# pcubillos/pyratbay

Measured on AMD Instinct MI355X. Metric: spectra/sec (1e5 wavenumbers x 80 layers), higher is better.
Workload: dtype f64; 1 GPU; 1e5 wavenumbers x 80 layers, 1e5 synthetic lines, transit; nwave=100001, nlayers=80, nlines=100000, wnosamp=180, voigt_grid=nlor=100 ndop=50 extent=300 cutoff=25, voigt_table_bytes=1448022784, parallelism=single GPU, 2 independent spectra in flight on 2 HIP streams, ranks=1, priming_spectra_in_init=32

## Files before the change

### include/pbhip.h

```cpp
#ifndef PBHIP_H
#define PBHIP_H

#include <stdint.h>

#ifdef __cplusplus
extern "C" {
#endif

#define PB_OK 0
#define PB_ERR_ARG (-1)
#define PB_ERR_HIP (-2)
#define PB_ERR_UNSUPPORTED (-3)
#define PB_ERR_NOMEM (-4)

const char *pb_last_error(void);
int pb_version(void);
int pb_device_count(int *count);
int pb_set_device(int device);

typedef struct pb_timer pb_timer;

int pb_timer_create(pb_timer **out, int max_stages);
int pb_timer_start(pb_timer *t, const char *first_stage, void *stream);
int pb_timer_mark(pb_timer *t, const char *name, const char *next_stage, void *stream);
// ... 42 lines not shown
int pb_lbl_set_isoiext(pb_lbl *p, const int32_t *isoiext_h);
int pb_lbl_set_ethresh(pb_lbl *p, double ethresh);
int pb_lbl_set_gather_mode(pb_lbl *p, int mode);
int pb_lbl_last_gather_mode(const pb_lbl *p, int *mode);
int pb_lbl_set_concurrency(pb_lbl *p, int n);
int pb_lbl_set_record_budget(pb_lbl *p, int64_t bytes);
int pb_lbl_last_chunks(const pb_lbl *p, int *chunks);
int pb_lbl_extinction(pb_lbl *p, double *ext_d, int64_t wbegin, int64_t wcount,
                      const double *temp_d, const double *dens_d, const double *isoz_d,
                      int64_t z_iso_stride, int64_t z_layer_stride, int nlayers, int add,
                      void *stream);
int pb_lbl_last_state(pb_lbl *p, int32_t *ofactor_h, double *kmax_h, int nlayers,
                      int nrows, void *stream);
int pb_lbl_last_layer_kinds(pb_lbl *p, int32_t *resident_h, int32_t *block_h, int nlayers,
                            void *stream);
int pb_lbl_extinction_begin(pb_lbl *p, double *ext_d, int64_t wbegin, int64_t wcount,
                            const double *temp_d, const double *dens_d, const double *isoz_d,
                            int64_t z_iso_stride, int64_t z_layer_stride, int nlayers, int add,
                            void *stream);
int pb_lbl_kmax_buffer(pb_lbl *p, void **kmax_d, int64_t *count);
int pb_lbl_extinction_end(pb_lbl *p, void *stream);
int pb_lbl_last_work(pb_lbl *p, int64_t work[3], void *stream);
int pb_lbl_last_table_samples(pb_lbl *p, int64_t *samples, void *stream);
int pb_lbl_timing_begin(pb_lbl *p, int max_launches);
int pb_lbl_timing_end(pb_lbl *p, double *total_ms, int *launches);
void pb_lbl_destroy(pb_lbl *p);

int pb_interp_ec(double *extinction_d, const double *etable_d, const double *ttable_d,
                 const double *temperatures_d, const double *density_d, int nmol,
                 int ntemp, int nlayers, int nwave, int lay1, int lay2, int per_mol,
// ... 550 lines not shown
```

### pyratbay_amd/_capi.py

```python
import ctypes as C
import os

import numpy as np

_HERE = os.path.dirname(os.path.abspath(__file__))
LIBPATH = os.environ.get('PB_LIBPBHIP') or os.path.join(_HERE, 'libpbhip.so')

PB_OK = 0


class PbError(RuntimeError):
    pass


_lib = None

vp = C.c_void_p
i32, i64, u64, f64 = C.c_int, C.c_int64, C.c_uint64, C.c_double

_PROTOS = {
    'pb_version': [],
    'pb_device_count': [C.POINTER(C.c_int)],
    'pb_set_device': [i32],
    'pb_timer_create': [C.POINTER(vp), i32],
# ... 19 lines not shown
    'pb_lbl_create': [C.POINTER(vp), vp, vp, vp, i32, vp, i32, vp, vp, i32, vp, vp, vp, vp,
                      i32, f64, f64, i32, i32],
    'pb_lbl_set_isoiext': [vp, vp],
    'pb_lbl_set_ethresh': [vp, f64],
    'pb_lbl_set_gather_mode': [vp, i32],
    'pb_lbl_set_concurrency': [vp, i32],
    'pb_lbl_set_record_budget': [vp, i64],
    'pb_lbl_last_chunks': [vp, C.POINTER(i32)],
    'pb_lbl_last_gather_mode': [vp, C.POINTER(i32)],
    'pb_lbl_extinction': [vp, vp, i64, i64, vp, vp, vp, i64, i64, i32, i32, vp],
    'pb_lbl_extinction_begin': [vp, vp, i64, i64, vp, vp, vp, i64, i64, i32, i32, vp],
    'pb_lbl_kmax_buffer': [vp, C.POINTER(vp), C.POINTER(i64)],
    'pb_lbl_extinction_end': [vp, vp],
    'pb_lbl_last_state': [vp, vp, vp, i32, i32, vp],
    'pb_lbl_last_layer_kinds': [vp, vp, vp, i32, vp],
    'pb_lbl_last_work': [vp, C.POINTER(i64 * 3), vp],
    'pb_lbl_last_table_samples': [vp, C.POINTER(i64), vp],
    'pb_lbl_timing_begin': [vp, i32],
    'pb_lbl_timing_end': [vp, C.POINTER(f64), C.POINTER(i32)],
    'pb_lbl_destroy': [vp],
    'pb_interp_ec': [vp, vp, vp, vp, vp, i32, i32, i32, i32, i32, i32, i32, vp],
    'pb_interp_ec_set': [vp, vp, vp, vp, vp, i32, i32, i32, i32, i32, i32, i32, vp],
    'pb_transit_path': [vp, vp, i32, i32, i32, vp],
    'pb_iso_partition': [vp, i64, i64, vp, i64, vp, i32, vp, i32, vp, vp],
    'pb_resample_cross_section': [vp, vp, vp, vp, vp, vp, vp, i32, i32, i32, i32, i32, i32, i32,
                                  i32, vp],
    'pb_interp_ec_batch_work_doubles': [i32, i32],
    'pb_interp_ec_batch_plan': [vp, i32, i32, i32, i32, i32, i32, i32],
    'pb_interp_ec_batch': [vp, vp, vp, vp, vp, vp, i32, i32, i32, i32, i32, vp],
    'pb_transit_work_doubles': [i32, i32, i32, i32, i32],
# ... 107 lines not shown
    'pb_lbl_set_dyn_predict': [vp, i32],
    'pb_table_transit_supported': [i32, i32, i32, i32, i32, i32],
    'pb_table_transit_work_doubles': [i32, i32, i32, i32, i32],
    'pb_table_transit_batch': [vp, vp, vp, vp, vp, vp, vp, f64, i32, i32, f64, i32, i32, i32, i32,
                               i32, vp, vp],
}
_RESTYPES = {'pb_transit_work_doubles': C.c_int64, 'pb_two_stream_batch_work_doubles': C.c_int64,
             'pb_two_stream_net_work_doubles': C.c_int64, 'pb_two_stream_net_parts': C.c_int,
             'pb_weighted_quantiles_work_doubles': C.c_int64,
             'pb_lm_work_doubles': C.c_int64,
             'pb_weighted_quantiles_resident_rows': C.c_int,
             'pb_band_contribution_work_doubles': C.c_int64,
             'pb_interp_ec_batch_work_doubles': C.c_int64,
             'pb_interp_ec_batch_cont_work_doubles': C.c_int64, 'pb_table_transit_work_doubles': C.c_int64,
             'pb_table_transit_supported': C.c_int, 'pb_voigt_destroy': None, 'pb_lines_destroy': None, 'pb_lbl_destroy': None,
             'pb_voigt_device_bytes': i64, 'pb_timer_destroy': None}
_NO_CHECK = set(_RESTYPES) | {'pb_version', 'pb_roctx_available'}


def exported_names():
    return sorted(list(_PROTOS) + ['pb_last_error'])


def experiments():
    return hasattr(lib(), 'pb_table_transit_batch')


def _preload_torch_hip_runtime():
    import torch
    cand = os.path.join(os.path.dirname(torch.__file__), 'lib', 'libamdhip64.so')
    if os.path.exists(cand):
# ... 62 lines not shown
```

### pyratbay_amd/csrc/pb_ext_args.h

```cpp
#pragma once

#include <cstdint>

#include "pb_common.h"
#include "pb_internal.h"

namespace pbx {

#ifdef PB_EXPERIMENTS
constexpr bool kExp = true;
#else
constexpr bool kExp = false;
#endif

constexpr int kBlock = 256;
constexpr int kChunks = 2;
constexpr int kLaneSamples = 2;
constexpr int kChunk = 64 * kLaneSamples;
constexpr int kWaveSpan = kChunks * kChunk;
constexpr int kTile = 4 * kWaveSpan;
constexpr int kRecs = 4;
static_assert(kTile <= kPmPad, "table padding must cover one tile");
static_assert(kTile < 65536, "window coordinates are packed in 16 bits");

constexpr int kLongLenBits = 14;
constexpr int kChunkRow = 1024;
constexpr int kRecLayers = 4;

constexpr int kBinSamples = 256;
constexpr int kStagePad = 256;
constexpr int kStageSpan = 256;
constexpr int kStageRowMax = 1024;

constexpr int kStagedWaves = 8;
constexpr int kStagedThreads = kStagedWaves * 64;
constexpr int64_t kStagedSub = kStagedWaves * kStageSpan;

constexpr int kResWaves = 8;
constexpr int kResThreads = kResWaves * 64;
constexpr int kResStrips = 2;
constexpr int kResTile = kResThreads * kResStrips;
constexpr int kResCapDefault = 8192;
static_assert(kResTile < 65536, "window coordinates are packed in 16 bits");

constexpr int kWvTile = 2048;
constexpr int kWvRowMax = 384;

// ... 22 lines not shown
    const int32_t *psize;
    const int32_t *pindex;
    const double *doppler;
    const double *lorentz;
    int ndop, nlor, osamp;
    const double *lwn, *elow, *gf;
    const int32_t *lid;
    const int32_t *gfirst, *gcount, *giown;
    const int64_t *iso_gstart;
    const int32_t *ph_first, *ph_count, *ph_iown;
    const int64_t *ph_start;
    const int32_t *ph_bin;
    int ph_nbins;
    int rowcap;
    int rowlds;
    const int32_t *ph_iso;
    const int32_t *giso;
    const int32_t *rk_first, *rk_count, *rk_iown, *rk_iso;
    const double *rk_lwn, *rk_elow, *rk_gf;
    const double *g_lead;
    int use_records;
    int64_t ngroups;
    int64_t rec_flo, rec_fhi;
    int kmax_local;
    const int32_t *wm_lo[2];
    const int32_t *wm_off[2];
    int wm_n[2];
    int wm_lds;
    int64_t wm_total[2];
    int32_t *ls_resident;
// ... 211 lines not shown
```

### pyratbay_amd/csrc/pb_ext_gather.hip

```cpp
#include <algorithm>
#include <climits>
#include <cmath>
#include <vector>

#include "pb_ext_plan.h"

using namespace pbx;

namespace {

template <int RS, int NW>
__global__ __launch_bounds__(NW * 64) void k_ext_resample(LblArgs a)
{
    constexpr int NT = NW * 64;
    constexpr int kTileRS = (NW / RS) * kWaveSpan;
    static_assert(NW % RS == 0, "wavefronts must divide evenly into record shares");
    __shared__ double s_k[NT];
    __shared__ unsigned s_off[NT];
    __shared__ unsigned s_win[NT];

    int tile, layer;
    decode_block(a, tile, layer);
    if (layer < 0 || (a.res_cap > 0 && a.ls_resident[layer]))
        return;
// ... 164 lines not shown
            }
        }
    }
    double *dst = a.ext + ((int64_t)layer * a.nrows + row) * a.wcount + (t0 - a.wbegin);
#pragma unroll
    for (int s = 0; s < kChunks; s++) {
        const int j = rlo + s * kChunk + 2 * lane;
        if (j < rhi)
            dst[j] = acc[s][0];
        if (j + 1 < rhi)
            dst[j + 1] = acc[s][1];
    }
}


template <int NW, int S, bool kDma, int kProbe = 0, int kIssue = 0>
__global__ __launch_bounds__(NW * 64, 8) void k_ext_staged(LblArgs a)
{
    constexpr int kThreads = NW * 64;
    constexpr int kSub = NW * kStageSpan;
    constexpr int kT = S * kSub;
    constexpr int kRowRegs = (kStageRowMax + kThreads - 1) / kThreads;
    static_assert(kT < 65536, "window coordinates are packed in 16 bits");
    extern __shared__ __align__(16) unsigned char smem[];
    const int osamp = a.osamp;
    double *s_row = reinterpret_cast<double *>(smem);
    struct __align__(16) Rec {
        double k;
        int qoff;
        unsigned win;
    };
// ... 27 lines not shown
            zsplit = e & 0xff;
        } else {
            layer = a.nlayers - 1 - unit / a.nsplit;
            zsplit = unit % a.nsplit;
        }
    }
    if (layer < 0 || (a.res_cap > 0 && a.ls_resident[layer]) || (a.wave_cap > 0 && a.ls_wave[layer]))
        return;
    const int nsp = a.tsplit ? a.tsplit[tile] : a.lsplit ? a.lsplit[layer] : a.nsplit;
    if (zsplit >= nsp)
        return;
    const int row = blockIdx.y;
    const int tid = threadIdx.x;
    const int lane = tid & 63;
    const int wave = __builtin_amdgcn_readfirstlane(tid >> 6);
    unsigned long long pc[21] = {0, 0, 0, 0, 0, 0, 0, 0, 0, 0, 0, 0, 0, 0, 0, 0, 0, 0, 0, 0, 0};
    auto tick = [&]() -> unsigned long long {
        if constexpr (kProbe == 4)
            return (unsigned long long)__builtin_amdgcn_s_memtime();
        return 0ull;
    };
    unsigned long long real_birth = 0;
    if constexpr (kProbe == 4) {
        real_birth = (unsigned long long)__builtin_amdgcn_s_memrealtime();
        const unsigned long long c0 = tick();
        const unsigned long long c1 = tick();
        const unsigned long long c2 = tick();
        pc[16] = (c2 - c0) + 0 * c1;
        pc[17] = 1;
    }
    const unsigned long long t_birth = tick();
// ... 19 lines not shown
    if (a.accumulate) {
#pragma unroll
        for (int u = 0; u < S; u++)
#pragma unroll
            for (int c = 0; c < 4; c++) {
                const int j = rlo + u * kSub + c * 64 + lane;
                if (j < tlen)
                    acc[u][c] = dst[j];
            }
    }
    for (int i = tid; i < kNB * rowspan + kStagePad; i += kThreads)
        s_row[i] = 0.0;

    double ring[kDma ? 1 : 2 * kRowRegs];
    int rowlim = a.rowlds;
    const unsigned row_lds0 = (unsigned)(size_t)(__attribute__((address_space(3))) char *)(
        reinterpret_cast<char *>(s_row + kStagePad));
    auto dma_desc = [&](unsigned long long d, int buf, int c_lo, int c_hi,
                        unsigned long long tref = 0) {
        const unsigned dlo = (unsigned)__builtin_amdgcn_readfirstlane((int)d);
        const unsigned dhi = (unsigned)__builtin_amdgcn_readfirstlane((int)(d >> 32));
        const long long first = ((long long)(dhi & 0xffu) << 32) | dlo;
        const int len = (int)((dhi >> 8) & 0xfffu), mlo = (int)(dhi >> 20);
        const unsigned long long base = (unsigned long long)(a.pm + first);
        typedef int v4i __attribute__((ext_vector_type(4)));
        v4i rsrc;
        rsrc.x = __builtin_amdgcn_readfirstlane((int)base);
        rsrc.y = __builtin_amdgcn_readfirstlane((int)((base >> 32) & 0xffffu));
        rsrc.z = __builtin_amdgcn_readfirstlane(len * 8);
        rsrc.w = 0x00020000;
        int voff = (2 * lane - (mlo & ~1)) * 8;
        unsigned dst = (unsigned)__builtin_amdgcn_readfirstlane((int)(row_lds0 + buf * rowspan * 8));
        if constexpr (kProbe == 4) {
            if (tref)
                pc[20] += tick() - tref;
        }
        voff += 1024 * c_lo;
        dst += 1024 * (unsigned)c_lo;
        for (int c = c_lo; c < c_hi && c * 128 < rowlim; c++) {
            unsigned keep;
            asm volatile("s_nop 4\n\t"
                         "s_mov_b32 %0, m0\n\t"
                         "s_mov_b32 m0, %1\n\t"
                         "s_nop 0\n\t"
                         "buffer_load_dwordx4 %2, %3, 0 offen lds\n\t"
                         "s_mov_b32 m0, %0"
                         : "=&s"(keep)
// ... 56 lines not shown
        const int64_t flo = t0 * osamp - reach, fhi = (tend - 1) * osamp + reach;

        __syncthreads();
        const int cell0 = a.li_ilor[li] * a.ndop;
        for (int d = tid; d < a.ndop; d += kThreads) {
            s_cbase[d] = a.pm_base[cell0 + d];
            s_csize[d] = a.psize[cell0 + d];
            s_cstride[d] = a.pm_stride[cell0 + d];
        }
        {
            const int lim = min(a.rowlds, a.li_rowmax[li]);
            if (lim != rowlim) {
                for (int i = tid; i < kNB * rowspan + kStagePad; i += kThreads)
                    s_row[i] = 0.0;
                rowlim = lim;
            }
        }
        const int nch = a.nch_max > 1
                            ? (min(a.rowcap, a.li_rowmax[li]) + kChunkRow - 1) / kChunkRow
                            : 1;
        const int nvirt = osamp * nch;
        const int per = (nvirt + kThreads - 1) / kThreads;
        int mine = 0;
        for (int r = 0; r < per; r++) {
            const int pv = tid * per + r;
            const int p = pv / nch, c = pv - p * nch;
            if (pv < nvirt && ((nsp > 1 && p * nsp / osamp != zsplit) ||
                               iso * osamp + p < a.key_lo || iso * osamp + p >= a.key_hi)) {
                s_phs[pv] = 0;
                s_cum[pv] = 0;
// ... 199 lines not shown
                            hi = mid;
                        else
                            lo = mid + 1;
                    }
                    hits[u] = slo < tlen ? (unsigned)first | ((unsigned)(lo - first) << 16) : 0u;
                }
            };
            auto walk = [&](int sg, int buf) {
                if ((sg & 63) == 0) {
                    const unsigned long long tf = tick();
                    find_hits(sg);
                    pc[3] += tick() - tf;
                }
                bool any = false;
                const char *rowp = reinterpret_cast<const char *>(
                    s_row + kStagePad + buf * rowspan + rlo + lane);
#pragma unroll
                for (int u = 0; u < S; u++) {
                    const unsigned h = (unsigned)__builtin_amdgcn_readlane((int)hits[u], sg & 63);
                    if (h < 0x10000u)
                        continue;
                    if constexpr (kProbe == 4) {
                        pc[12] += h >> 16;
                        any = true;
                    }
                    const int first = (int)(h & 0xffff);
                    const int last = first + (int)(h >> 16);
                    const char *rs = rowp + (size_t)u * kSub * 8;
                    const double2 *recs = reinterpret_cast<const double2 *>(s_rec);
                    auto visit = [&](const double2 raw) {
                        const double k = raw.x;
// ... 92 lines not shown
                    unsigned long long dn = s_desc[min(nseg - 1, 1)];
                    dma_desc(s_desc[0], 0, wave * kPer, wave * kPer + kPer);
                    __builtin_amdgcn_s_waitcnt(0x0f70);
                    __syncthreads();
                    for (int sg = 0; sg < nseg; sg++) {
                        const unsigned long long dcur = dn;
                        dn = s_desc[min(nseg - 1, sg + 2)];
                        if (sg + 1 < nseg)
                            dma_desc(dcur, (sg + 1) & 1, wave * kPer, wave * kPer + kPer);
                        walk(sg, sg & 1);
                        __builtin_amdgcn_s_waitcnt(0x0f70);
                        __syncthreads();
                    }
                    continue;
                }
                unsigned long long ta = tick();
                if (wave == 0)
                    dma_row(0, 0);
                __builtin_amdgcn_s_waitcnt(0x0f70);
                __syncthreads();
                if constexpr (kProbe == 4) {
                    const unsigned long long tb = tick();
                    pc[8] += tb - ta;
                    ta = tb;
                }
                for (int sg = 0; sg < nseg; sg++) {
                    if (sg + 1 < nseg && wave == ((sg + 1) & (NW - 1)))
                        dma_row(sg + 1, (sg + 1) & 1, ta);
                    if constexpr (kProbe == 4) {
                        const unsigned long long tb = tick();
                        if (sg + 1 < nseg && wave == ((sg + 1) & (NW - 1))) {
                            pc[4] += tb - ta;
                            pc[19] += 1;
                        } else {
                            pc[18] += tb - ta;
                        }
                        ta = tb;
                        const unsigned long long f0 = pc[3];
                        walk(sg, sg & 1);
                        const unsigned long long tc = tick();
                        pc[5] += (tc - ta) - (pc[3] - f0);
                        __builtin_amdgcn_s_waitcnt(0x0f70);
                        const unsigned long long td = tick();
                        pc[6] += td - tc;
                        __syncthreads();
                        ta = tick();
                        pc[7] += ta - td;
                        pc[10] += 1;
                        continue;
                    }
                    walk(sg, sg & 1);
                    __builtin_amdgcn_s_waitcnt(0x0f70);
                    __syncthreads();
                }
            } else if (nseg > 0) {
                run(std::integral_constant<int, 2>(), std::integral_constant<int, kRowRegs>());
            }
        }
    }

    const unsigned long long t_out = tick();
#pragma unroll
    for (int u = 0; u < S; u++) {
#pragma unroll
        for (int c = 0; c < 4; c++) {
            const int j = rlo + u * kSub + c * 64 + lane;
            if (j < tlen)
                dst[j] = acc[u][c];
        }
    }
    if constexpr (kProbe == 4) {
        const unsigned long long t_end = tick();
        pc[14] += t_end - t_out;
        pc[9] = t_end - t_birth;
        pc[15] = (unsigned long long)__builtin_amdgcn_s_memrealtime() - real_birth;
        if (lane == 0 && a.probe)
            for (int i = 0; i < 21; i++)
                atomicAdd(&a.probe[(int64_t)layer * 24 + i], pc[i]);
    }
}

__global__ __launch_bounds__(kResThreads) void k_ext_resident(LblArgs a)
{
    extern __shared__ __align__(16) unsigned char smem[];
    struct __align__(16) Rec {
        double k;
        int off;
        unsigned win;
    };
    double *s_prof = reinterpret_cast<double *>(smem);
    const int zslot = a.res_cap;
    Rec *s_rec = reinterpret_cast<Rec *>(s_prof + a.res_cap + 2);
// ... 326 lines not shown
        return;
    const int64_t j = (int64_t)blockIdx.x * kBlock + threadIdx.x;
    if (j >= per_layer)
        return;
    const int64_t i = (int64_t)layer * per_layer + j;
    double v = ext[i];
    for (int p = 0; p < nparts; p++)
        v += part[(int64_t)p * n + i];
    ext[i] = v;
}

}

namespace pbx {

GatherKernel staged_kernel(int S, bool dma)
{
    return dma ? (S == 4   ? k_ext_staged<kStagedWaves, 4, true>
                  : S == 2 ? k_ext_staged<kStagedWaves, 2, true>
                           : k_ext_staged<kStagedWaves, 1, true>)
               : (S == 4   ? k_ext_staged<kStagedWaves, 4, false>
                  : S == 2 ? k_ext_staged<kStagedWaves, 2, false>
                           : k_ext_staged<kStagedWaves, 1, false>);
}

int allow_lds(const void *kern, size_t lds)
{
    if (lds > 64 * 1024)
        PB_HIP(hipFuncSetAttribute(kern, hipFuncAttributeMaxDynamicSharedMemorySize, (int)lds));
    return PB_OK;
}

// ... 97 lines not shown

static int exp_stage_probe_begin(LblArgs &a, const GatherPlan &g, const Tuning &tn,
                                 GatherKernel *kern, hipStream_t s)
{
    const int e = tn.stage_probe;
    if (g.S != 2 || !g.dma)
        return PB_OK;
    if (e >= 1 && e <= 3)
        *kern = e == 1   ? k_ext_staged<kStagedWaves, 2, true, 1>
                : e == 2 ? k_ext_staged<kStagedWaves, 2, true, 2>
                         : k_ext_staged<kStagedWaves, 2, true, 3>;
    if (e >= 11 && e <= 12)
        *kern = e == 11 ? k_ext_staged<kStagedWaves, 2, true, 0, 1>
                        : k_ext_staged<kStagedWaves, 2, true, 0, 2>;
    if (e == 4) {
        *kern = k_ext_staged<kStagedWaves, 2, true, 4>;
        PB_HIP(hipMalloc(&a.probe, (size_t)a.nlayers * 24 * 8));
        PB_HIP(hipMemsetAsync(a.probe, 0, (size_t)a.nlayers * 24 * 8, s));
    }
    return PB_OK;
}

static int exp_stage_probe_end(LblArgs &a, hipStream_t s)
{
    if (!a.probe)
        return PB_OK;
    std::vector<unsigned long long> h((size_t)a.nlayers * 24);
    PB_HIP(hipMemcpyAsync(h.data(), a.probe, h.size() * 8, hipMemcpyDeviceToHost, s));
    std::vector<int32_t> rowmax((size_t)a.nlayers * a.niso);
    PB_HIP(hipMemcpyAsync(rowmax.data(), a.li_rowmax, rowmax.size() * 4,
                          hipMemcpyDeviceToHost, s));
    PB_HIP(hipStreamSynchronize(s));
    (void)hipFree(a.probe);
    a.probe = nullptr;
    for (int layer = 0; layer < a.nlayers; layer++) {
        fprintf(stderr, "STAGE_PROBE layer %d rowmax %d :", layer,
                rowmax[(size_t)layer * a.niso]);
        for (int i = 0; i < 21; i++)
            fprintf(stderr, " %llu", h[(size_t)layer * 24 + i]);
        fprintf(stderr, "\n");
    }
    return PB_OK;
}
#else
static inline int exp_stage_probe_begin(LblArgs &, const GatherPlan &, const Tuning &,
                                        GatherKernel *, hipStream_t) { return PB_OK; }
static inline int exp_stage_probe_end(LblArgs &, hipStream_t) { return PB_OK; }
#endif

static int tile_split_table(pb_lbl *p, const LblArgs &a, const GatherPlan &g, const Tuning &tn,
                            int nsplit, hipStream_t s)
{
    const pb_voigt *v = p->voigt;
// ... 108 lines not shown
    }
    if (deep > 0) {
        if (int rc = layer_split_table(p, nlayers, nsplit, deep, deep_split, s))
            return rc;
        a.unit_tab = p->d_unit_tab;
        a.lsplit = p->d_lsplit;
        a.nunits = p->ut_units;
    }
    const int nunits = deep > 0 ? p->ut_units : nlayers * nsplit;
    a.nsplit = nsplit;
    if (int rc = ensure_part(p, a, deep > 0 ? deep_split : nsplit, s))
        return rc;
    a.ntiles = pb::div_up(wcount, g.S * kStagedSub);
    const int unit_groups = (nunits + 7) / 8;
    dim3 grid((unsigned)(8 * a.ntiles * unit_groups), a.nrows);
    GatherKernel kern = staged_kernel(g.S, g.dma);
    if (int rc = exp_stage_probe_begin(a, g, tn, &kern, s))
        return rc;
    if (int rc = allow_lds(reinterpret_cast<const void *>(kern), g.lds))
        return rc;
    if (int rc = exp_launch_wave(a, nunits, s))
        return rc;
    kern<<<grid, kStagedThreads, g.lds, s>>>(a);
    if (int rc = exp_stage_probe_end(a, s))
        return rc;
    const int32_t *resident = a.res_cap > 0 ? a.ls_resident : nullptr;
    const int64_t per_layer = (int64_t)a.nrows * wcount, n = nlayers * per_layer;
    if (deep > 0) {
        PB_LAUNCH_CHECK();
        dim3 cgrid((unsigned)pb::div_up(per_layer, kBlock), nlayers);
        k_combine_layer_parts<<<cgrid, kBlock, 0, s>>>(a.ext, p->part, p->d_lsplit, per_layer, n,
// ... 55 lines not shown
```

### pyratbay_amd/csrc/pb_ext_plan.h

```cpp
#pragma once

#include <vector>

#include "pb_ext_args.h"

struct pb_lbl {
    pb_voigt *voigt = nullptr;
    pb_lines *lines = nullptr;
    int nwave = 0, nmol = 0, niso = 0, ndivs = 0, max_layers = 0, resolution = 0;
    int nrows_sep = 1;
    double cutoff = 0, ethresh = 0, wnstep = 0, wn0 = 0;
    std::vector<int32_t> isoiext;
    double *d_wn = nullptr, *d_molrad = nullptr, *d_molmass = nullptr, *d_isomass = nullptr,
           *d_isoratio = nullptr;
    int32_t *d_divisors = nullptr, *d_isoimol = nullptr, *d_isoiext = nullptr;
    int32_t *ls_ofactor = nullptr, *ls_scale = nullptr, *li_ilor = nullptr, *li_hmax = nullptr;
    int32_t *li_rowmax = nullptr, *li_hlo = nullptr, *li_hhi = nullptr;
    int64_t *ls_dnwn = nullptr;
    double *ls_dwnstep = nullptr, *li_alphad = nullptr, *li_dens = nullptr, *li_z = nullptr;
    double *ls_quot = nullptr;
    double *li_invz = nullptr;
    unsigned long long *kmax_bits = nullptr;
    int kmax_rows = 0;
    int32_t *ph_first = nullptr, *ph_count = nullptr, *ph_iown = nullptr;
// ... 31 lines not shown
    bool res_look_pending = false;
    size_t record_budget = (size_t)96 << 30;
    int last_chunks = 0;
    int32_t *d_unit_tab = nullptr, *d_lsplit = nullptr;
    size_t ut_bytes = 0, ls_bytes = 0;
    int32_t *d_tsplit = nullptr;
    int32_t *pos2ph = nullptr;
    bool ts_sparse = false;
    int64_t ts_key[4] = {-1, -1, -1, -1};
    int ts_max = 0;
    size_t ts_bytes = 0;
    int ut_key[4] = {-1, -1, -1, -1};
    int ut_units = 0;
    int concurrency = 1;
    int gather_mode = 0;
    int last_gather = 0;
    double stage_threshold = 8.0;
    std::vector<hipEvent_t> ev;
    int ev_used = 0;
    int64_t *unit_cap = nullptr;
    size_t unit_cap_bytes = 0;
    int64_t cap_key[5] = {-1, -1, -1, -1, -1};
    pbx::VRec *vrec = nullptr;
    pbx::VSeg *vseg = nullptr;
    int32_t *vrnd = nullptr;
    size_t vrec_alloc = 0;
    pbx::UnitHdr *uhdr = nullptr;
    size_t uhdr_bytes = 0;
    struct Pending {
        double *ext;
// ... 33 lines not shown
    std::vector<int32_t> h_ofactor, h_ilor, h_divisors, h_isoimol, h_isoiext0;
    std::vector<double> h_wn, h_molrad, h_molmass, h_isomass, h_isoratio;
};

namespace pbx {

using Call = pb_lbl::Pending;
using GatherKernel = void (*)(LblArgs);

struct Tuning {
    int experiment = 0;
    bool dma = true;
    bool no_long_rows = false;
    int stage_s = 0;
    int stage_split = 0;
    bool poison = false;
    bool budget_set = false;
    size_t budget = 0;
    bool rec_soa = false;
    int wave = -1;
    bool res_dyn_off = false;
    bool rec_layers_1 = false;
    bool no_window_map = false;
    size_t wm_lds_cap = 48 * 1024;
    int scatter_t = 512;
    int rounds_geom = 2;
    bool deep_set = false;
    double deep_frac = 0.0;
    int deep_factor = 2;
    bool tile_split_off = false;
// ... 28 lines not shown
    int fmt = 0;
};

int64_t group_reach(const pb_voigt *v, double cutoff, double ownstep);
int64_t groups_in_reach(const pb_lines *l, int niso, int64_t flo, int64_t fhi);
int ensure_bytes(void **ptr, size_t *have, size_t need, hipStream_t s, bool sync_first,
                 const char *what);
int64_t plane_bytes(const LblArgs &a);
int cap_split_to_planes(int n, int64_t plane, int least = 1);
int ensure_part(pb_lbl *p, LblArgs &a, int nplanes, hipStream_t s);
int lbl_extinction(pb_lbl *p, const Call &c, void *stream, int phase);
int launch_layer_state(const LblArgs &a, hipStream_t s);
int launch_kmax(const LblArgs &a, hipStream_t s);
size_t records_lds(const LblArgs &a, int per);
int launch_records(const LblArgs &a, int fmt, int per, dim3 grid, size_t lds, hipStream_t s);
GatherKernel staged_kernel(int S, bool dma);
int allow_lds(const void *kern, size_t lds);
int launch_staged(pb_lbl *p, LblArgs &a, const GatherPlan &g, const Tuning &tn, hipStream_t s);
int launch_global(LblArgs &a, const Tuning &tn, hipStream_t s);
int launch_resident(LblArgs &a, hipStream_t s);
int launch_linterp(LblArgs &a, hipStream_t s);
int lbl_resolution_dyn(pb_lbl *p, LblArgs &a, const Call &c, const Tuning &tn, hipStream_t s);

#ifdef PB_EXPERIMENTS
int exp_launch_scatter(LblArgs &a, const Tuning &tn, hipStream_t s);
int exp_launch_rounds(pb_lbl *p, LblArgs &a, const GatherPlan &g, const Tuning &tn, hipStream_t s);
int exp_launch_wave(const LblArgs &a, int nunits, hipStream_t s);
#else
static inline int exp_launch_scatter(LblArgs &, const Tuning &, hipStream_t) { return PB_OK; }
static inline int exp_launch_rounds(pb_lbl *, LblArgs &, const GatherPlan &, const Tuning &,
                                    hipStream_t) { return PB_OK; }
// ... 5 lines not shown
```

### pyratbay_amd/csrc/pb_ext_resolution.hip

```cpp
#include <algorithm>
#include <vector>

#include "pb_ext_plan.h"

using namespace pbx;

namespace {

__global__ __launch_bounds__(kBlock) void k_ext_linterp(LblArgs a)
{
    struct __align__(16) RecA {
        double k;
        int64_t start;
    };
    struct __align__(16) RecB {
        int inoff, half2, mn, mx;
    };
    __shared__ RecA s_ra[kBlock + 4];
    __shared__ RecB s_rb[kBlock + 4];

    int tile, layer;
    decode_block(a, tile, layer);
    if (layer < 0)
        return;
// ... 181 lines not shown
    for (int32_t x : p->h_divisors)
        if (x <= f && f % x == 0)
            divs.push_back(x);
    const int64_t dn = 1 + (l->onwn - 1) / f;
    std::vector<double> wn((size_t)dn);
    for (int64_t i = 0; i < dn; i++)
        wn[(size_t)i] = l->own0 + (double)(i * f) * l->ownstep;
    rc = pb_lbl_create(&d.plan, d.voigt, p->lines, wn.data(), (int)dn, divs.data(),
                       (int)divs.size(), p->h_molrad.data(), p->h_molmass.data(), p->nmol,
                       p->h_isoimol.data(), p->h_isomass.data(), p->h_isoratio.data(),
                       p->h_isoiext0.data(), p->niso, p->cutoff, p->ethresh, 0, p->max_layers);
    if (rc)
        return rc;
    if (!getenv("PB_GATHER"))
        d.plan->gather_mode = 2;
    p->dyn.push_back(d);
    *out = &p->dyn.back();
    return PB_OK;
}

int lbl_resolution_dyn(pb_lbl *p, LblArgs &a, const Call &c, const Tuning &tn, hipStream_t s)
{
    const pb_lines *l = p->lines;
    const int nlayers = c.nlayers;
    const int64_t wbegin = c.wbegin, wcount = c.wcount;
    PB_REQUIRE(l->onwn < (1LL << 30), "pb_lbl_extinction: fine grid of %lld samples exceeds 2^30",
               (long long)l->onwn);
    if (int rc = launch_layer_state(a, s))
        return rc;
    const size_t nstate = (size_t)nlayers * (1 + p->niso);
// ... 290 lines not shown
```

### pyratbay_amd/csrc/pb_extinction.hip

```cpp
#include <algorithm>
#include <climits>
#include <cmath>
#include <cstdlib>
#include <new>
#include <vector>

#include "pb_ext_plan.h"

using namespace pbx;

namespace {

__global__ __launch_bounds__(kBlock) void k_poison_records(Rec16 *rec16, int64_t n16, Rec32 *rec32,
                                                          int64_t n32, double *rec_k,
                                                          int32_t *rec_i32, int64_t nsoa)
{
    const int64_t stride = (int64_t)gridDim.x * kBlock;
    for (int64_t i = (int64_t)blockIdx.x * kBlock + threadIdx.x; i < n16; i += stride) {
        Rec16 r;
        r.k = 1e300;
        r.ulo = 0;
        r.lc = 0xfffu;
        rec16[i] = r;
    }
// ... 382 lines not shown
static Tuning read_tuning()
{
    Tuning t;
    auto is_zero = [](const char *name) {
        const char *e = getenv(name);
        return e && atoi(e) == 0;
    };
    if (const char *e = getenv("PB_EXPERIMENT"))
        t.experiment = atoi(e);
    t.dma = !is_zero("PB_STAGE_DMA");
    t.no_long_rows = getenv("PB_NO_LONG_ROWS") != nullptr;
    if (const char *e = getenv("PB_STAGE_S"))
        t.stage_s = atoi(e) >= 4 ? 4 : atoi(e) >= 2 ? 2 : 1;
    if (const char *e = getenv("PB_STAGE_SPLIT"))
        t.stage_split = std::max(1, std::min(8, atoi(e)));
    if (const char *e = getenv("PB_POISON_RECORDS"))
        t.poison = atoi(e) != 0;
    if (const char *e = getenv("PB_RECORD_BUDGET")) {
        t.budget_set = true;
        t.budget = (size_t)atoll(e);
    }
    t.rec_soa = getenv("PB_REC_SOA") != nullptr;
    t.res_dyn_off = is_zero("PB_RES_DYN");
    if (const char *e = getenv("PB_REC_LAYERS"))
        t.rec_layers_1 = atoi(e) == 1;
    t.no_window_map = getenv("PB_NO_WINDOW_MAP") != nullptr;
    if (const char *e = getenv("PB_WM_LDS_CAP"))
        t.wm_lds_cap = (size_t)atol(e);
    if (const char *e = getenv("PB_STAGE_DEEP")) {
        t.deep_set = true;
// ... 418 lines not shown

static int run_chunked(pb_lbl *p, LblArgs &a, const GatherPlan &g, hipStream_t s)
{
    const int nlayers = a.nlayers;
    if (int rc = launch_kmax(a, s))
        return rc;
    const bool timed = p->ev_used + 2 <= (int)p->ev.size();
    if (timed)
        PB_HIP(hipEventRecord(p->ev[p->ev_used], s));
    const int per = kRecLayers;
    const size_t rlds = records_lds(a, per) + 8;
    PB_REQUIRE(rlds <= 64 * 1024, "pb_lbl_extinction: %zu B of LDS for the record kernel", rlds);
    a.ntiles = pb::div_up(a.wcount, g.S * kStagedSub);
    const int unit_groups = (nlayers + 7) / 8;
    dim3 ggrid((unsigned)(8 * a.ntiles * unit_groups), a.nrows);
    GatherKernel kern = staged_kernel(g.S, g.dma);
    if (int rc = allow_lds(reinterpret_cast<const void *>(kern), g.lds))
        return rc;
    for (size_t c = 0; c < g.chunks.size(); c++) {
        a.grp_lo = g.chunks[c].g_lo;
        a.grp_hi = g.chunks[c].g_hi;
        a.rec_pitch = std::max<int64_t>(1, a.grp_hi - a.grp_lo);
        a.key_lo = g.chunks[c].key_lo;
        a.key_hi = g.chunks[c].key_hi;
        a.accumulate = c > 0 ? 1 : 0;
        if (a.grp_hi > a.grp_lo) {
            dim3 rgrid(pb::div_up(a.grp_hi - a.grp_lo, kBlock), pb::div_up(nlayers, per));
            if (int rc = launch_records(a, g.fmt, per, rgrid, rlds, s))
                return rc;
        }
        kern<<<ggrid, kStagedThreads, g.lds, s>>>(a);
// ... 121 lines not shown
        if (int rc = pb_voigt_ensure_flat(p->voigt, s))
            return rc;
    const Tuning tn = read_tuning();
    LblArgs a = fill_args(p, c);
    a.kmax_local = phase != 0 ? 1 : 0;
    a.experiment = tn.experiment;

    GatherPlan g = plan_gather(p, a, tn, phase);
    resident_probe(p, g, s, phase);
    if (g.rc)
        return g.rc;
    const bool chunked = !g.chunks.empty();
    p->last_chunks = (int)g.chunks.size();
    a.nch_max = g.nch_max;
    a.rowlds = g.rowlds;
    a.res_cap = g.resident && !chunked ? p->res_cap : 0;
    if (int rc = bind_records(p, a, g, tn, s))
        return rc;

    bool dyn_fall = false;
    if (p->resolution && p->gather_mode == 6 && phase == 0 && l->ngroups > 0 &&
        l->onwn > 2 * (int64_t)p->voigt->osamp && !tn.res_dyn_off) {
        const int rc = lbl_resolution_dyn(p, a, c, tn, s);
        if (!(rc == PB_ERR_UNSUPPORTED && p->dyn_runs == 0)) {
            if (rc != PB_OK || !p->dyn_fallback)
                return rc;
            dyn_fall = true;
            a.lskip = p->d_ok;
        }
    }
// ... 118 lines not shown
        PB_HIP(hipMemcpy(kmax_h, p->kmax_bits, (size_t)nlayers * nrows * 8,
                         hipMemcpyDeviceToHost));
    return PB_OK;
}

int pb_lbl_last_layer_kinds(pb_lbl *p, int32_t *resident_h, int32_t *block_h, int nlayers,
                            void *stream)
{
    PB_REQUIRE(p, "pb_lbl_last_layer_kinds: null handle");
    PB_REQUIRE(nlayers >= 1 && nlayers <= p->max_layers, "pb_lbl_last_layer_kinds: bad sizes");
    PB_HIP(hipStreamSynchronize(pb::as_stream(stream)));
    if (resident_h)
        PB_HIP(hipMemcpy(resident_h, p->ls_resident, (size_t)nlayers * 4, hipMemcpyDeviceToHost));
    if (block_h)
        PB_HIP(hipMemcpy(block_h, p->ls_block, (size_t)nlayers * 4, hipMemcpyDeviceToHost));
    return PB_OK;
}

#ifdef PB_EXPERIMENTS
int pb_lbl_last_wave_layers(pb_lbl *p, int32_t *wave_h, int nlayers, void *stream)
{
    PB_REQUIRE(p && wave_h, "pb_lbl_last_wave_layers: null pointer");
    PB_REQUIRE(nlayers >= 1 && nlayers <= p->max_layers, "pb_lbl_last_wave_layers: bad sizes");
    PB_HIP(hipStreamSynchronize(pb::as_stream(stream)));
    if (p->last_args.wave_cap > 0)
        PB_HIP(hipMemcpy(wave_h, p->ls_wave, (size_t)nlayers * 4, hipMemcpyDeviceToHost));
    else
        memset(wave_h, 0, (size_t)nlayers * 4);
    return PB_OK;
}
// ... 124 lines not shown
```

### pyratbay_amd/lbl.py

```python
import ctypes as C

import numpy as np
import torch

from ._capi import call, hptr, f64h, i32h
from ._device import _ptr, _stream, dev, require_gpu


class VoigtTable:

    def __init__(self, handle, nlor, ndop, lorentz, doppler, osamp):
        self._h = handle
        self.nlor, self.ndop, self.osamp = nlor, ndop, osamp
        self.lorentz, self.doppler = lorentz, doppler
        size = np.zeros((nlor, ndop), np.int32)
        index = np.zeros((nlor, ndop), np.int32)
        n = C.c_int64(0)
        call('pb_voigt_meta', self._h, hptr(size), hptr(index), C.byref(n))
        self.size, self.index, self.nprofile = size, index, n.value

    @classmethod
    def build(cls, lorentz, doppler, size, ownstep, osamp, keep_flat=False):
        require_gpu()
        lorentz, doppler = f64h(lorentz), f64h(doppler)
# ... 233 lines not shown
        return None if n.value < 0 else int(n.value)

    def last_state(self, nlayers, rows):
        ofactor = np.zeros(nlayers, np.int32)
        kmax = np.zeros((nlayers, rows))
        call('pb_lbl_last_state', self._h, hptr(ofactor), hptr(kmax), nlayers, rows,
             _stream())
        return ofactor, kmax

    def last_layer_kinds(self, nlayers):
        resident = np.zeros(nlayers, np.int32)
        block = np.zeros(nlayers, np.int32)
        call('pb_lbl_last_layer_kinds', self._h, hptr(resident), hptr(block), nlayers, _stream())
        return resident, block

    def last_wave_layers(self, nlayers):
        wave = np.zeros(nlayers, np.int32)
        call('pb_lbl_last_wave_layers', self._h, hptr(wave), nlayers, _stream())
        return wave

    def set_dyn_predict(self, on=True):
        call('pb_lbl_set_dyn_predict', self._h, int(bool(on)))

    def dyn_stats(self):
        st = np.zeros(3, np.int64)
        call('pb_lbl_dyn_stats', self._h, hptr(st))
        return tuple(int(v) for v in st)

    def close(self):
        if self._h:
# ... 9 lines not shown
```

Before: 1123 spectra/s.

## Stage multiple DMA rows per barrier step in staged gather kernel

```diff
diff --git a/include/pbhip.h b/include/pbhip.h
--- a/include/pbhip.h
+++ b/include/pbhip.h
@@ -80,6 +80,8 @@
                       int nrows, void *stream);
 int pb_lbl_last_layer_kinds(pb_lbl *p, int32_t *resident_h, int32_t *block_h, int nlayers,
                             void *stream);
+int pb_lbl_rows_per_step(int rowlds, int rowlim, int *pitch);
+int pb_lbl_last_rows_per_step(pb_lbl *p, int32_t *rows_h, int nlayers, int niso, void *stream);
 int pb_lbl_extinction_begin(pb_lbl *p, double *ext_d, int64_t wbegin, int64_t wcount,
                             const double *temp_d, const double *dens_d, const double *isoz_d,
                             int64_t z_iso_stride, int64_t z_layer_stride, int nlayers, int add,
diff --git a/pyratbay_amd/_capi.py b/pyratbay_amd/_capi.py
--- a/pyratbay_amd/_capi.py
+++ b/pyratbay_amd/_capi.py
@@ -57,6 +57,8 @@
     'pb_lbl_extinction_end': [vp, vp],
     'pb_lbl_last_state': [vp, vp, vp, i32, i32, vp],
     'pb_lbl_last_layer_kinds': [vp, vp, vp, i32, vp],
+    'pb_lbl_rows_per_step': [i32, i32, C.POINTER(i32)],
+    'pb_lbl_last_rows_per_step': [vp, vp, i32, i32, vp],
     'pb_lbl_last_work': [vp, C.POINTER(i64 * 3), vp],
     'pb_lbl_last_table_samples': [vp, C.POINTER(i64), vp],
     'pb_lbl_timing_begin': [vp, i32],
@@ -194,7 +196,8 @@
              'pb_interp_ec_batch_work_doubles': C.c_int64,
              'pb_interp_ec_batch_cont_work_doubles': C.c_int64, 'pb_table_transit_work_doubles': C.c_int64,
              'pb_table_transit_supported': C.c_int, 'pb_voigt_destroy': None, 'pb_lines_destroy': None, 'pb_lbl_destroy': None,
-             'pb_voigt_device_bytes': i64, 'pb_timer_destroy': None}
+             'pb_voigt_device_bytes': i64, 'pb_timer_destroy': None,
+             'pb_lbl_rows_per_step': C.c_int}
 _NO_CHECK = set(_RESTYPES) | {'pb_version', 'pb_roctx_available'}
 
 
diff --git a/pyratbay_amd/csrc/pb_ext_args.h b/pyratbay_amd/csrc/pb_ext_args.h
--- a/pyratbay_amd/csrc/pb_ext_args.h
+++ b/pyratbay_amd/csrc/pb_ext_args.h
@@ -31,6 +31,25 @@
 constexpr int kStagePad = 256;
 constexpr int kStageSpan = 256;
 constexpr int kStageRowMax = 1024;
+constexpr int kStageRowsMax = 2;
+constexpr int kStageRowsDefault = kStageRowsMax;
+
+struct StageSlots {
+    int pitch, rows;
+};
+__host__ __device__ inline StageSlots stage_slots(int rowlds, int rowlim, int cap = kStageRowsMax)
+{
+    const int area = 2 * (rowlds + kStagePad);
+    const int pitch = (rowlim + kStagePad) & ~1;
+    int rows = area / pitch / 2;
+    if (rows > cap)
+        rows = cap;
+    if (rows > kStageRowsMax)
+        rows = kStageRowsMax;
+    if (rows < 2)
+        return {(rowlds + kStagePad) & ~1, 1};
+    return {pitch, rows};
+}
 
 constexpr int kStagedWaves = 8;
 constexpr int kStagedThreads = kStagedWaves * 64;
@@ -83,6 +102,7 @@
     int ph_nbins;
     int rowcap;
     int rowlds;
+    int rows_cap;
     const int32_t *ph_iso;
     const int32_t *giso;
     const int32_t *rk_first, *rk_count, *rk_iown, *rk_iso;
diff --git a/pyratbay_amd/csrc/pb_ext_gather.hip b/pyratbay_amd/csrc/pb_ext_gather.hip
--- a/pyratbay_amd/csrc/pb_ext_gather.hip
+++ b/pyratbay_amd/csrc/pb_ext_gather.hip
@@ -202,7 +202,7 @@
 }
 
 
-template <int NW, int S, bool kDma, int kProbe = 0, int kIssue = 0>
+template <int NW, int S, bool kDma, int kProbe = 0, int kIssue = 0, int kRows = 1>
 __global__ __launch_bounds__(NW * 64, 8) void k_ext_staged(LblArgs a)
 {
     constexpr int kThreads = NW * 64;
@@ -260,7 +260,7 @@
     const int tid = threadIdx.x;
     const int lane = tid & 63;
     const int wave = __builtin_amdgcn_readfirstlane(tid >> 6);
-    unsigned long long pc[21] = {0, 0, 0, 0, 0, 0, 0, 0, 0, 0, 0, 0, 0, 0, 0, 0, 0, 0, 0, 0, 0};
+    unsigned long long pc[22] = {0, 0, 0, 0, 0, 0, 0, 0, 0, 0, 0, 0, 0, 0, 0, 0, 0, 0, 0, 0, 0, 0};
     auto tick = [&]() -> unsigned long long {
         if constexpr (kProbe == 4)
             return (unsigned long long)__builtin_amdgcn_s_memtime();
@@ -310,6 +310,10 @@
 
     double ring[kDma ? 1 : 2 * kRowRegs];
     int rowlim = a.rowlds;
+    constexpr bool kMulti = kDma && kIssue == 0 && kRows > 1;
+    int pitch = rowspan, nrow = 1;
+    static_assert(kRows <= kStageRowsMax && kStageRowsMax <= NW,
+                  "a wavefront requests at most one row of a step");
     const unsigned row_lds0 = (unsigned)(size_t)(__attribute__((address_space(3))) char *)(
         reinterpret_cast<char *>(s_row + kStagePad));
     auto dma_desc = [&](unsigned long long d, int buf, int c_lo, int c_hi,
@@ -326,7 +330,7 @@
         rsrc.z = __builtin_amdgcn_readfirstlane(len * 8);
         rsrc.w = 0x00020000;
         int voff = (2 * lane - (mlo & ~1)) * 8;
-        unsigned dst = (unsigned)__builtin_amdgcn_readfirstlane((int)(row_lds0 + buf * rowspan * 8));
+        unsigned dst = (unsigned)__builtin_amdgcn_readfirstlane((int)(row_lds0 + buf * (kMulti ? pitch : rowspan) * 8));
         if constexpr (kProbe == 4) {
             if (tref)
                 pc[20] += tick() - tref;
@@ -413,6 +417,11 @@
                 for (int i = tid; i < kNB * rowspan + kStagePad; i += kThreads)
                     s_row[i] = 0.0;
                 rowlim = lim;
+                if constexpr (kMulti) {
+                    const StageSlots sl = stage_slots(a.rowlds, lim, min(kRows, a.rows_cap));
+                    pitch = sl.pitch;
+                    nrow = sl.rows;
+                }
             }
         }
         const int nch = a.nch_max > 1
@@ -642,7 +651,7 @@
                 }
                 bool any = false;
                 const char *rowp = reinterpret_cast<const char *>(
-                    s_row + kStagePad + buf * rowspan + rlo + lane);
+                    s_row + kStagePad + buf * (kMulti ? pitch : rowspan) + rlo + lane);
 #pragma unroll
                 for (int u = 0; u < S; u++) {
                     const unsigned h = (unsigned)__builtin_amdgcn_readlane((int)hits[u], sg & 63);
@@ -765,9 +774,59 @@
                     }
                     continue;
                 }
+                if constexpr (!kMulti) {
+                    unsigned long long ta = tick();
+                    if (wave == 0)
+                        dma_row(0, 0);
+                    __builtin_amdgcn_s_waitcnt(0x0f70);
+                    __syncthreads();
+                    if constexpr (kProbe == 4) {
+                        const unsigned long long tb = tick();
+                        pc[8] += tb - ta;
+                        ta = tb;
+                    }
+                    for (int sg = 0; sg < nseg; sg++) {
+                        if (sg + 1 < nseg && wave == ((sg + 1) & (NW - 1)))
+                            dma_row(sg + 1, (sg + 1) & 1, ta);
+                        if constexpr (kProbe == 4) {
+                            const unsigned long long tb = tick();
+                            if (sg + 1 < nseg && wave == ((sg + 1) & (NW - 1))) {
+                                pc[4] += tb - ta;
+                                pc[19] += 1;
+                            } else {
+                                pc[18] += tb - ta;
+                            }
+                            ta = tb;
+                            const unsigned long long f0 = pc[3];
+                            walk(sg, sg & 1);
+                            const unsigned long long tc = tick();
+                            pc[5] += (tc - ta) - (pc[3] - f0);
+                            __builtin_amdgcn_s_waitcnt(0x0f70);
+                            const unsigned long long td = tick();
+                            pc[6] += td - tc;
+                            __syncthreads();
+                            ta = tick();
+                            pc[7] += ta - td;
+                            pc[10] += 1;
+                            pc[21] += 1;
+                            continue;
+                        }
+                        walk(sg, sg & 1);
+                        __builtin_amdgcn_s_waitcnt(0x0f70);
+                        __syncthreads();
+                    }
+                    continue;
+                }
+                auto step_end = [&](int s0) { return min(min(s0 + nrow, nseg), (s0 | 63) + 1); };
+                auto request = [&](int s0, int s1, int slot0, unsigned long long tref) {
+                    const int g = s0 + ((wave - s0) & (NW - 1));
+                    if (g < s1)
+                        dma_row(g, slot0 + (g - s0), tref);
+                    return g < s1;
+                };
                 unsigned long long ta = tick();
-                if (wave == 0)
-                    dma_row(0, 0);
+                int sg = 0, se = step_end(0), half = 0;
+                request(0, se, 0, 0);
                 __builtin_amdgcn_s_waitcnt(0x0f70);
                 __syncthreads();
                 if constexpr (kProbe == 4) {
@@ -775,12 +834,12 @@
                     pc[8] += tb - ta;
                     ta = tb;
                 }
-                for (int sg = 0; sg < nseg; sg++) {
-                    if (sg + 1 < nseg && wave == ((sg + 1) & (NW - 1)))
-                        dma_row(sg + 1, (sg + 1) & 1, ta);
+                while (sg < nseg) {
+                    const int sn = step_end(se);
+                    const bool asked = request(se, sn, (half ^ 1) * nrow, ta);
                     if constexpr (kProbe == 4) {
                         const unsigned long long tb = tick();
-                        if (sg + 1 < nseg && wave == ((sg + 1) & (NW - 1))) {
+                        if (asked) {
                             pc[4] += tb - ta;
                             pc[19] += 1;
                         } else {
@@ -788,7 +847,8 @@
                         }
                         ta = tb;
                         const unsigned long long f0 = pc[3];
-                        walk(sg, sg & 1);
+                        for (int g = sg; g < se; g++)
+                            walk(g, half * nrow + (g - sg));
                         const unsigned long long tc = tick();
                         pc[5] += (tc - ta) - (pc[3] - f0);
                         __builtin_amdgcn_s_waitcnt(0x0f70);
@@ -798,11 +858,17 @@
                         ta = tick();
                         pc[7] += ta - td;
                         pc[10] += 1;
-                        continue;
-                    }
-                    walk(sg, sg & 1);
-                    __builtin_amdgcn_s_waitcnt(0x0f70);
-                    __syncthreads();
+                        pc[21] += (unsigned long long)(se - sg);
+                    } else {
+                        (void)asked;
+                        for (int g = sg; g < se; g++)
+                            walk(g, half * nrow + (g - sg));
+                        __builtin_amdgcn_s_waitcnt(0x0f70);
+                        __syncthreads();
+                    }
+                    sg = se;
+                    se = sn;
+                    half ^= 1;
                 }
             } else if (nseg > 0) {
                 run(std::integral_constant<int, 2>(), std::integral_constant<int, kRowRegs>());
@@ -826,7 +892,7 @@
         pc[9] = t_end - t_birth;
         pc[15] = (unsigned long long)__builtin_amdgcn_s_memrealtime() - real_birth;
         if (lane == 0 && a.probe)
-            for (int i = 0; i < 21; i++)
+            for (int i = 0; i < 22; i++)
                 atomicAdd(&a.probe[(int64_t)layer * 24 + i], pc[i]);
     }
 }
@@ -1183,8 +1249,13 @@
 
 namespace pbx {
 
-GatherKernel staged_kernel(int S, bool dma)
-{
+GatherKernel staged_kernel(int S, bool dma, int rows)
+{
+    constexpr int R = kStageRowsMax;
+    if (dma && rows > 1)
+        return S == 4   ? k_ext_staged<kStagedWaves, 4, true, 0, 0, R>
+               : S == 2 ? k_ext_staged<kStagedWaves, 2, true, 0, 0, R>
+                        : k_ext_staged<kStagedWaves, 1, true, 0, 0, R>;
     return dma ? (S == 4   ? k_ext_staged<kStagedWaves, 4, true>
                   : S == 2 ? k_ext_staged<kStagedWaves, 2, true>
                            : k_ext_staged<kStagedWaves, 1, true>)
@@ -1312,7 +1383,8 @@
         *kern = e == 11 ? k_ext_staged<kStagedWaves, 2, true, 0, 1>
                         : k_ext_staged<kStagedWaves, 2, true, 0, 2>;
     if (e == 4) {
-        *kern = k_ext_staged<kStagedWaves, 2, true, 4>;
+        *kern = a.rows_cap > 1 ? k_ext_staged<kStagedWaves, 2, true, 4, 0, kStageRowsMax>
+                               : k_ext_staged<kStagedWaves, 2, true, 4>;
         PB_HIP(hipMalloc(&a.probe, (size_t)a.nlayers * 24 * 8));
         PB_HIP(hipMemsetAsync(a.probe, 0, (size_t)a.nlayers * 24 * 8, s));
     }
@@ -1334,7 +1406,7 @@
     for (int layer = 0; layer < a.nlayers; layer++) {
         fprintf(stderr, "STAGE_PROBE layer %d rowmax %d :", layer,
                 rowmax[(size_t)layer * a.niso]);
-        for (int i = 0; i < 21; i++)
+        for (int i = 0; i < 22; i++)
             fprintf(stderr, " %llu", h[(size_t)layer * 24 + i]);
         fprintf(stderr, "\n");
     }
@@ -1473,7 +1545,7 @@
     a.ntiles = pb::div_up(wcount, g.S * kStagedSub);
     const int unit_groups = (nunits + 7) / 8;
     dim3 grid((unsigned)(8 * a.ntiles * unit_groups), a.nrows);
-    GatherKernel kern = staged_kernel(g.S, g.dma);
+    GatherKernel kern = staged_kernel(g.S, g.dma, a.rows_cap);
     if (int rc = exp_stage_probe_begin(a, g, tn, &kern, s))
         return rc;
     if (int rc = allow_lds(reinterpret_cast<const void *>(kern), g.lds))
diff --git a/pyratbay_amd/csrc/pb_ext_plan.h b/pyratbay_amd/csrc/pb_ext_plan.h
--- a/pyratbay_amd/csrc/pb_ext_plan.h
+++ b/pyratbay_amd/csrc/pb_ext_plan.h
@@ -69,6 +69,7 @@
     int ut_units = 0;
     int concurrency = 1;
     int gather_mode = 0;
+    bool dyn_child = false;
     int last_gather = 0;
     double stage_threshold = 8.0;
     std::vector<hipEvent_t> ev;
@@ -132,6 +133,7 @@
     bool no_long_rows = false;
     int stage_s = 0;
     int stage_split = 0;
+    int stage_rows = 0;
     bool poison = false;
     bool budget_set = false;
     size_t budget = 0;
@@ -190,7 +192,7 @@
 int launch_kmax(const LblArgs &a, hipStream_t s);
 size_t records_lds(const LblArgs &a, int per);
 int launch_records(const LblArgs &a, int fmt, int per, dim3 grid, size_t lds, hipStream_t s);
-GatherKernel staged_kernel(int S, bool dma);
+GatherKernel staged_kernel(int S, bool dma, int rows);
 int allow_lds(const void *kern, size_t lds);
 int launch_staged(pb_lbl *p, LblArgs &a, const GatherPlan &g, const Tuning &tn, hipStream_t s);
 int launch_global(LblArgs &a, const Tuning &tn, hipStream_t s);
diff --git a/pyratbay_amd/csrc/pb_ext_resolution.hip b/pyratbay_amd/csrc/pb_ext_resolution.hip
--- a/pyratbay_amd/csrc/pb_ext_resolution.hip
+++ b/pyratbay_amd/csrc/pb_ext_resolution.hip
@@ -219,6 +219,7 @@
         return rc;
     if (!getenv("PB_GATHER"))
         d.plan->gather_mode = 2;
+    d.plan->dyn_child = true;
     p->dyn.push_back(d);
     *out = &p->dyn.back();
     return PB_OK;
diff --git a/pyratbay_amd/csrc/pb_extinction.hip b/pyratbay_amd/csrc/pb_extinction.hip
--- a/pyratbay_amd/csrc/pb_extinction.hip
+++ b/pyratbay_amd/csrc/pb_extinction.hip
@@ -420,6 +420,8 @@
         t.stage_s = atoi(e) >= 4 ? 4 : atoi(e) >= 2 ? 2 : 1;
     if (const char *e = getenv("PB_STAGE_SPLIT"))
         t.stage_split = std::max(1, std::min(8, atoi(e)));
+    if (const char *e = getenv("PB_STAGE_ROWS"))
+        t.stage_rows = std::max(1, std::min(kStageRowsMax, atoi(e)));
     if (const char *e = getenv("PB_POISON_RECORDS"))
         t.poison = atoi(e) != 0;
     if (const char *e = getenv("PB_RECORD_BUDGET")) {
@@ -868,7 +870,7 @@
     a.ntiles = pb::div_up(a.wcount, g.S * kStagedSub);
     const int unit_groups = (nlayers + 7) / 8;
     dim3 ggrid((unsigned)(8 * a.ntiles * unit_groups), a.nrows);
-    GatherKernel kern = staged_kernel(g.S, g.dma);
+    GatherKernel kern = staged_kernel(g.S, g.dma, a.rows_cap);
     if (int rc = allow_lds(reinterpret_cast<const void *>(kern), g.lds))
         return rc;
     for (size_t c = 0; c < g.chunks.size(); c++) {
@@ -1020,6 +1022,9 @@
     p->last_chunks = (int)g.chunks.size();
     a.nch_max = g.nch_max;
     a.rowlds = g.rowlds;
+    a.rows_cap = g.dma && g.nch_max == 1
+                     ? (tn.stage_rows ? tn.stage_rows : p->dyn_child ? 1 : kStageRowsDefault)
+                     : 1;
     a.res_cap = g.resident && !chunked ? p->res_cap : 0;
     if (int rc = bind_records(p, a, g, tn, s))
         return rc;
@@ -1168,6 +1173,32 @@
         PB_HIP(hipMemcpy(resident_h, p->ls_resident, (size_t)nlayers * 4, hipMemcpyDeviceToHost));
     if (block_h)
         PB_HIP(hipMemcpy(block_h, p->ls_block, (size_t)nlayers * 4, hipMemcpyDeviceToHost));
+    return PB_OK;
+}
+
+int pb_lbl_rows_per_step(int rowlds, int rowlim, int *pitch)
+{
+    const StageSlots sl = stage_slots(rowlds, rowlim);
+    if (pitch)
+        *pitch = sl.pitch;
+    return sl.rows;
+}
+
+int pb_lbl_last_rows_per_step(pb_lbl *p, int32_t *rows_h, int nlayers, int niso, void *stream)
+{
+    PB_REQUIRE(p && rows_h, "pb_lbl_last_rows_per_step: null pointer");
+    PB_REQUIRE(nlayers >= 1 && nlayers <= p->max_layers && niso == p->niso,
+               "pb_lbl_last_rows_per_step: bad sizes");
+    PB_HIP(hipStreamSynchronize(pb::as_stream(stream)));
+    const size_t n = (size_t)nlayers * niso;
+    const LblArgs &a = p->last_args;
+    if ((p->last_gather & 7) != 2 || a.rows_cap <= 1) {
+        std::fill(rows_h, rows_h + n, 1);
+        return PB_OK;
+    }
+    PB_HIP(hipMemcpy(rows_h, p->li_rowmax, n * 4, hipMemcpyDeviceToHost));
+    for (size_t i = 0; i < n; i++)
+        rows_h[i] = stage_slots(a.rowlds, std::min(a.rowlds, rows_h[i]), a.rows_cap).rows;
     return PB_OK;
 }
 
diff --git a/pyratbay_amd/lbl.py b/pyratbay_amd/lbl.py
--- a/pyratbay_amd/lbl.py
+++ b/pyratbay_amd/lbl.py
@@ -271,6 +271,11 @@
         call('pb_lbl_last_layer_kinds', self._h, hptr(resident), hptr(block), nlayers, _stream())
         return resident, block
 
+    def last_rows_per_step(self, nlayers, niso):
+        rows = np.zeros((nlayers, niso), np.int32)
+        call('pb_lbl_last_rows_per_step', self._h, hptr(rows), nlayers, niso, _stream())
+        return rows
+
     def last_wave_layers(self, nlayers):
         wave = np.zeros(nlayers, np.int32)
         call('pb_lbl_last_wave_layers', self._h, hptr(wave), nlayers, _stream())
```

Result: faster. 1144 spectra/s, median of 6 (+1.9%).
